# pyannote/pyannote-audio

Measured on AMD Instinct MI355X. Metric: audio-hours/sec (real-time factor) for speaker-diarization-3.1 pipeline, higher is better.
Workload: dtype f32

## Files before the change

### pyannote-audio_amd/csrc/seg_frontend.hip

```cpp
#include "common.h"

namespace pa {

__global__ __launch_bounds__(256) void k_row_stats(const float* __restrict__ x, long row_stride,
                                                    long total_len, int len, float eps,
                                                    float* __restrict__ mean_out,
                                                    float* __restrict__ rstd_out) {
  __shared__ float red[4];
  const long base = (long)blockIdx.x * row_stride;
  long avail = total_len - base;
  int valid = avail >= len ? len : (avail > 0 ? (int)avail : 0);
  const float* row = x + base;
  float s = 0.f;
  for (int i = threadIdx.x; i < valid; i += 256) s += row[i];
  const float mean = block_sum<4>(s, red) / (float)len;
  float q = 0.f;
  for (int i = threadIdx.x; i < valid; i += 256) {
    float d = row[i] - mean;
    q += d * d;
  }
  float var = block_sum<4>(q, red);
  var += (float)(len - valid) * mean * mean;
  var /= (float)len;
  if (threadIdx.x == 0) {
    mean_out[blockIdx.x] = mean;
    rstd_out[blockIdx.x] = 1.0f / sqrtf(var + eps);
  }
}

constexpr int SINC_PT = 128;
constexpr int SINC_XS = 30 * SINC_PT + 256;
constexpr int SINC_OS = SINC_PT + 4;
constexpr int SINC_T = 640;
constexpr float SINC_DEMOTE = 0.5f;

__device__ __forceinline__ float sinc_centre(float mean0, float rstd0) {
  return fabsf(mean0) * rstd0 > SINC_DEMOTE ? mean0 : 0.f;
}
__device__ __forceinline__ bool sinc_demoted(float mu, float rstd, float m0) {
  return fabsf(mu - m0) * rstd > SINC_DEMOTE;
}

template <bool RAW, int STR = 10>
__global__ __launch_bounds__(SINC_T) void k_sinc_fir_pool(
    const float* __restrict__ wav, long wav_len, long chunk_stride, int N, int stride, int P,
    const float* __restrict__ mean, const float* __restrict__ rstd, float gamma, float beta,
    const float* __restrict__ filt, float* __restrict__ out, int centred) {
  constexpr int XS_MAX = 3 * STR * SINC_PT + 256;
  extern __shared__ __attribute__((aligned(16))) float smem[];
  float* xs = smem;
  float* os = smem + XS_MAX;
  const int b = blockIdx.y;
  const int p0 = blockIdx.x * SINC_PT;
  const int tid = threadIdx.x, lane = tid & 63;
  const int w = (tid >> 6) % 5, half = (tid >> 6) / 5;
  constexpr int PS = RAW ? STR : 3 * STR;
  constexpr int XS = RAW ? STR * SINC_PT + 256 : XS_MAX;

  const long cbase = (long)b * chunk_stride;
  if (!RAW && centred && !sinc_demoted(mean[b], rstd[b], sinc_centre(mean[0], rstd[0]))) return;
  const float mu = RAW ? (centred ? sinc_centre(mean[0], rstd[0]) : 0.f) : mean[b], rs = RAW ? 1.f : rstd[b] * gamma;
  if (RAW) beta = 0.f;
  {
    constexpr int NS = (XS_MAX + SINC_T - 1) / SINC_T;
    float raw[NS];
#pragma unroll
    for (int k = 0; k < NS; ++k) {
      const int i = tid + SINC_T * k;
      const long g = cbase + PS * p0 + i;
      raw[k] = (i < XS && PS * p0 + i < N && g < wav_len) ? wav[g] : 0.f;
    }
#pragma unroll
    for (int k = 0; k < NS; ++k) {
      const int i = tid + SINC_T * k;
      if (i < XS) xs[i] = PS * p0 + i < N ? (raw[k] - mu) * rs + beta : 0.f;
    }
  }
  float fb[63];
#pragma unroll
  for (int kt = 0; kt < 63; ++kt) fb[kt] = filt[(w * 63 + kt) * 64 + lane];
  __syncthreads();

  const int i16 = lane & 15, kq = lane >> 4;
#pragma unroll 1
  for (int grp = half * (SINC_PT / 32); grp < (half + 1) * (SINC_PT / 32); ++grp) {
    f32x4 a0 = {0, 0, 0, 0}, a1 = {0, 0, 0, 0}, a2 = {0, 0, 0, 0};
    const float* xp = xs + PS * (16 * grp + i16) + kq;
#pragma unroll
    for (int kt = 0; kt < 63; ++kt) {
      a0 = MFMA16(xp[4 * kt], fb[kt], a0);
      if (!RAW) {
        a1 = MFMA16(xp[4 * kt + STR], fb[kt], a1);
        a2 = MFMA16(xp[4 * kt + 2 * STR], fb[kt], a2);
      }
    }
#pragma unroll
    for (int r = 0; r < 4; ++r) {
      const float v = RAW ? a0[r] : fmaxf(fmaxf(fabsf(a0[r]), fabsf(a1[r])), fabsf(a2[r]));
      os[(16 * w + i16) * SINC_OS + 16 * grp + 4 * kq + r] = v;
    }
  }
  __syncthreads();
  const int np = min(SINC_PT, P - p0);
  for (int i = tid; i < 80 * SINC_PT; i += SINC_T) {
    const int c = i / SINC_PT, p = i % SINC_PT;
    if (p < np) out[((long)b * 80 + c) * P + p0 + p] = os[c * SINC_OS + p];
  }
}

__global__ __launch_bounds__(128) void k_sinc_tapsum(const float* __restrict__ filt, float* __restrict__ S1) {
  const int f = threadIdx.x;
  if (f >= 80) return;
  double acc = 0.0;
  for (int kt = 0; kt < 63; ++kt)
    for (int q = 0; q < 4; ++q) acc += (double)filt[((f >> 4) * 63 + kt) * 64 + (f & 15) + 16 * q];
  S1[f] = (float)acc;
}

__global__ __launch_bounds__(256) void k_sinc_fix_pool(const float* __restrict__ S, long Pc, int Q, int P,
                                                        const float* __restrict__ mean,
                                                        const float* __restrict__ rstd, float gamma, float beta,
                                                        const float* __restrict__ S1, float* __restrict__ out,
                                                        int centred) {
  const int b = blockIdx.y, p = blockIdx.x * 256 + threadIdx.x;
  if (p >= P) return;
  const float m0 = centred ? sinc_centre(mean[0], rstd[0]) : 0.f;
  if (centred && sinc_demoted(mean[b], rstd[b], m0)) return;
  const float mu = mean[b] - m0, g = rstd[b] * gamma;
  const float* src = S + (long)b * Q + 3 * p;
  float* dst = out + (long)b * 80 * P + p;
#pragma unroll 8
  for (int f = 0; f < 80; ++f) {
    const float s1 = S1[f], off = beta * s1 - g * mu * s1;
    const float* row = src + (long)f * Pc;
    const float v0 = fabsf(fmaf(g, row[0], off)), v1 = fabsf(fmaf(g, row[1], off)), v2 = fabsf(fmaf(g, row[2], off));
    dst[(long)f * P] = fmaxf(fmaxf(v0, v1), v2);
  }
}

constexpr int CV_PT = 32;
constexpr int CV_XW = 112;
constexpr int CV_OS = CV_PT + 1;

template <int CIN>
__global__ __launch_bounds__(256) void k_conv5_pool(const float* __restrict__ xin, int Lin, int P,
                                                     const float* __restrict__ in_mean,
                                                     const float* __restrict__ in_rstd,
                                                     const float* __restrict__ gam,
                                                     const float* __restrict__ bet,
                                                     const float* __restrict__ wp,
                                                     const float* __restrict__ bias,
                                                     float* __restrict__ out) {
  constexpr int KT = 5 * CIN / 4;
  constexpr int KPT = CIN / 4;
  __shared__ __attribute__((aligned(16))) float xs[CIN * CV_XW];
  __shared__ float os[64 * CV_OS];
  const int b = blockIdx.y;
  const int p0 = blockIdx.x * CV_PT;
  const int tid = threadIdx.x, lane = tid & 63, w = tid >> 6;

  {
    static_assert(CIN % 20 == 0, "five channel rows per wave and trip");
    const int wu = __builtin_amdgcn_readfirstlane(w);
    const int q1 = lane + 64;
    const bool ok0 = 3 * p0 + lane < Lin;
    const bool ok1 = q1 < 3 * CV_PT + 4 && 3 * p0 + q1 < Lin;
#pragma unroll
    for (int j0 = 0; j0 < CIN / 4; j0 += 5) {
      float x0[5], x1[5], mu[5], sc[5], sh[5];
#pragma unroll
      for (int u = 0; u < 5; ++u) {
        const int c = wu + 4 * (j0 + u), row = b * CIN + c;
        const float* src = xin + (long)row * Lin + 3 * p0;
        x0[u] = ok0 ? src[lane] : 0.f;
        x1[u] = ok1 ? src[q1] : 0.f;
        mu[u] = in_mean[row];
        sc[u] = in_rstd[row] * gam[c];
        sh[u] = bet[c];
      }
#pragma unroll
      for (int u = 0; u < 5; ++u) {
        float* dst = xs + (wu + 4 * (j0 + u)) * CV_XW;
        dst[lane] = ok0 ? leaky_relu((x0[u] - mu[u]) * sc[u] + sh[u]) : 0.f;
        if (q1 < CV_XW) dst[q1] = ok1 ? leaky_relu((x1[u] - mu[u]) * sc[u] + sh[u]) : 0.f;
      }
    }
  }
  float wb[KT];
#pragma unroll
  for (int kt = 0; kt < KT; ++kt) wb[kt] = wp[(w * KT + kt) * 64 + lane];
  __syncthreads();

  const int i16 = lane & 15, kq = lane >> 4;
  const float bv = bias[16 * w + i16];
#pragma unroll 1
  for (int grp = 0; grp < CV_PT / 16; ++grp) {
    f32x4 a0 = {0, 0, 0, 0}, a1 = {0, 0, 0, 0}, a2 = {0, 0, 0, 0};
    const float* xp = xs + kq * CV_XW + 3 * (16 * grp + i16);
#pragma unroll
    for (int kt = 0; kt < KT; ++kt) {
      const int tap = kt / KPT, c4 = (kt % KPT) * 4;
      const float* q = xp + c4 * CV_XW + tap;
      a0 = MFMA16(q[0], wb[kt], a0);
      a1 = MFMA16(q[1], wb[kt], a1);
      a2 = MFMA16(q[2], wb[kt], a2);
    }
#pragma unroll
    for (int r = 0; r < 4; ++r) {
      float v = fmaxf(fmaxf(a0[r], a1[r]), a2[r]) + bv;
      os[(16 * w + i16) * CV_OS + 16 * grp + 4 * kq + r] = v;
    }
  }
  __syncthreads();
  const int np = min(CV_PT, P - p0);
  for (int i = tid; i < 60 * CV_PT; i += 256) {
    const int c = i / CV_PT, p = i % CV_PT;
    if (p < np) out[((long)b * 60 + c) * P + p0 + p] = os[c * CV_OS + p];
  }
}

__global__ __launch_bounds__(256) void k_norm_transpose(const float* __restrict__ xin, int B, int T,
                                                         const float* __restrict__ in_mean,
                                                         const float* __restrict__ in_rstd,
                                                         const float* __restrict__ gam,
                                                         const float* __restrict__ bet,
                                                         float* __restrict__ X0) {
  __shared__ float tile[64][65];
  const int b = blockIdx.y, t0 = blockIdx.x * 64;
  const int tid = threadIdx.x;
  for (int i = tid; i < 64 * 64; i += 256) {
    const int c = i >> 6, tt = i & 63;
    float v = 0.f;
    if (b < B && c < 60 && t0 + tt < T) {
      const int row = b * 60 + c;
      v = (xin[(long)row * T + t0 + tt] - in_mean[row]) * (in_rstd[row] * gam[c]) + bet[c];
      v = leaky_relu(v);
    }
    tile[c][tt] = v;
  }
  __syncthreads();
  const int bt = b >> 4, b16 = b & 15;
  for (int i = tid; i < 64 * 64; i += 256) {
    const int tt = i >> 6, c = i & 63;
    if (t0 + tt < T) X0[(((long)bt * T + t0 + tt) * 16 + b16) * 64 + c] = tile[c][tt];
  }
}

}

extern "C" {

int pa_row_stats(const float* x, long row_stride, long total_len, int rows, int len, float eps,
                 float* mean, float* rstd, void* stream) {
  if (rows <= 0) return 0;
  pa::ProfScope prof("k_row_stats", stream, 5.0 * rows * len, 8.0 * rows * len);
  hipLaunchKernelGGL(pa::k_row_stats, dim3(rows), dim3(256), 0, (hipStream_t)stream, x, row_stride,
                     total_len, len, eps, mean, rstd);
  PA_CHECK_LAUNCH("pa_row_stats");
  return 0;
}

int pa_sinc_fir_pool(const float* wav, long wav_len, long chunk_stride, int B, int N, int stride,
                     const float* mean, const float* rstd, float gamma, float beta,
                     const float* filt_packed, float* out, void* stream) {
  PA_REQUIRE(stride >= 1 && N >= 251, "pa_sinc_fir_pool: stride %d / %d samples", stride, N);
  const int L = (N - 251) / stride + 1;
  const int P = L / 3;
  if (B <= 0 || P <= 0) return 0;
  pa::ProfScope prof("k_sinc_fir_pool", stream, 2.0 * B * 80 * 251 * (3.0 * P),
                     4.0 * B * N + 4.0 * B * 80 * P);
#define PA_SINC_LAUNCH(S)                                                                                          \
  do {                                                                                                             \
    const size_t lds = (size_t)(3 * (S) * pa::SINC_PT + 256 + 80 * pa::SINC_OS) * sizeof(float);                     \
                         \
    (void)hipFuncSetAttribute((const void*)pa::k_sinc_fir_pool<false, S>, hipFuncAttributeMaxDynamicSharedMemorySize, \
                              (int)lds);                                                                           \
    hipLaunchKernelGGL((pa::k_sinc_fir_pool<false, S>), dim3(pa::cdiv(P, pa::SINC_PT), B), dim3(pa::SINC_T), lds,  \
                       (hipStream_t)stream, wav, wav_len, chunk_stride, N, stride, P, mean, rstd, gamma, beta,      \
                       filt_packed, out, 0);                                                                       \
  } while (0)
  switch (stride) {
    case 10: PA_SINC_LAUNCH(10); break;
    case 1: PA_SINC_LAUNCH(1); break;
    case 2: PA_SINC_LAUNCH(2); break;
    case 4: PA_SINC_LAUNCH(4); break;
    case 5: PA_SINC_LAUNCH(5); break;
    case 8: PA_SINC_LAUNCH(8); break;
    case 16: PA_SINC_LAUNCH(16); break;
    case 20: PA_SINC_LAUNCH(20); break;
    default:
      PA_REQUIRE(false, "pa_sinc_fir_pool: SincNet stride %d is not built (1, 2, 4, 5, 8, 10, 16, 20 are)", stride);
  }
#undef PA_SINC_LAUNCH
  PA_CHECK_LAUNCH("pa_sinc_fir_pool");
  return 0;
}

static int sinc_fir_span(const float* wav, long wav_len, long span, const float* mean0, const float* rstd0,
                         const float* filt_packed, float* S, void* stream) {
  if (span < 251) return 0;
  PA_REQUIRE(span <= 0x7fffffffL, "pa_sinc_fir_span: span of %ld samples is too long", span);
  const int Pc = (int)((span - 251) / 10 + 1);
  const size_t lds = (pa::SINC_XS + 80 * pa::SINC_OS) * sizeof(float);
  (void)hipFuncSetAttribute((const void*)pa::k_sinc_fir_pool<true>, hipFuncAttributeMaxDynamicSharedMemorySize,
                            (int)lds);
  pa::ProfScope prof("k_sinc_fir_span", stream, 2.0 * 80 * 251 * (double)Pc, 4.0 * span + 4.0 * 80 * Pc);
  hipLaunchKernelGGL(pa::k_sinc_fir_pool<true>, dim3(pa::cdiv(Pc, pa::SINC_PT), 1), dim3(pa::SINC_T), lds,
                     (hipStream_t)stream, wav, wav_len, 0L, (int)span, 10, Pc, mean0, rstd0, 1.f, 0.f, filt_packed, S,
                     mean0 != nullptr ? 1 : 0);
  PA_CHECK_LAUNCH("pa_sinc_fir_span");
  return 0;
}

int pa_sinc_fir_span(const float* wav, long wav_len, long span, const float* filt_packed, float* S, void* stream) {
  return sinc_fir_span(wav, wav_len, span, nullptr, nullptr, filt_packed, S, stream);
}

int pa_sinc_fir_span_centred(const float* wav, long wav_len, long span, const float* mean0, const float* rstd0,
                             const float* filt_packed, float* S, void* stream) {
  PA_REQUIRE(mean0 != nullptr && rstd0 != nullptr, "pa_sinc_fir_span_centred: the statistics of chunk 0 are missing");
  return sinc_fir_span(wav, wav_len, span, mean0, rstd0, filt_packed, S, stream);
}

int pa_sinc_fix_pool(const float* S, long Pc, int positions_per_chunk_step, int B, int P, const float* mean,
                     const float* rstd, float gamma, float beta, const float* filt_packed, float* tap_sums,
                     float* out, void* stream) {
  if (B <= 0 || P <= 0) return 0;
  pa::ProfScope prof("k_sinc_fix_pool", stream, 8.0 * B * 80 * 3.0 * P, 4.0 * B * 80 * 4.0 * P);
  hipLaunchKernelGGL(pa::k_sinc_tapsum, dim3(1), dim3(128), 0, (hipStream_t)stream, filt_packed, tap_sums);
  hipLaunchKernelGGL(pa::k_sinc_fix_pool, dim3(pa::cdiv(P, 256), B), dim3(256), 0, (hipStream_t)stream, S, Pc,
                     positions_per_chunk_step, P, mean, rstd, gamma, beta, (const float*)tap_sums, out, 0);
  PA_CHECK_LAUNCH("pa_sinc_fix_pool");
  return 0;
}

int pa_sinc_fix_pool_centred(const float* S, long Pc, int positions_per_chunk_step, int B, int P, const float* wav,
                             long wav_len, int N, const float* mean, const float* rstd, float gamma, float beta,
                             const float* filt_packed, float* tap_sums, float* out, void* stream) {
  if (B <= 0 || P <= 0) return 0;
  PA_REQUIRE(N >= 251 && P == ((N - 251) / 10 + 1) / 3, "pa_sinc_fix_pool_centred: %d pooled positions of %d samples",
             P, N);
  pa::ProfScope prof("k_sinc_fix_pool", stream, 8.0 * B * 80 * 3.0 * P, 4.0 * B * 80 * 4.0 * P);
  hipLaunchKernelGGL(pa::k_sinc_tapsum, dim3(1), dim3(128), 0, (hipStream_t)stream, filt_packed, tap_sums);
  hipLaunchKernelGGL(pa::k_sinc_fix_pool, dim3(pa::cdiv(P, 256), B), dim3(256), 0, (hipStream_t)stream, S, Pc,
                     positions_per_chunk_step, P, mean, rstd, gamma, beta, (const float*)tap_sums, out, 1);
  {
    const size_t lds = (pa::SINC_XS + 80 * pa::SINC_OS) * sizeof(float);
    (void)hipFuncSetAttribute((const void*)pa::k_sinc_fir_pool<false, 10>, hipFuncAttributeMaxDynamicSharedMemorySize,
                              (int)lds);
    hipLaunchKernelGGL((pa::k_sinc_fir_pool<false, 10>), dim3(pa::cdiv(P, pa::SINC_PT), B), dim3(pa::SINC_T), lds,
                       (hipStream_t)stream, wav, wav_len, 10L * positions_per_chunk_step, N, 10, P, mean, rstd, gamma,
                       beta, filt_packed, out, 1);
  }
  PA_CHECK_LAUNCH("pa_sinc_fix_pool_centred");
  return 0;
}

int pa_conv5_pool(const float* xin, int B, int cin, int Lin, const float* in_mean,
                  const float* in_rstd, const float* gam, const float* bet, const float* w_packed,
                  const float* bias64, float* out, void* stream) {
  const int P = (Lin - 4) / 3;
  if (B <= 0 || P <= 0) return 0;
  dim3 grid(pa::cdiv(P, pa::CV_PT), B);
  pa::ProfScope prof("k_conv5_pool", stream, 2.0 * B * 60 * cin * 5 * (3.0 * P),
                     4.0 * B * cin * Lin + 4.0 * B * 60 * P);
  if (cin == 80)
    hipLaunchKernelGGL(pa::k_conv5_pool<80>, grid, dim3(256), 0, (hipStream_t)stream, xin, Lin, P,
                       in_mean, in_rstd, gam, bet, w_packed, bias64, out);
  else if (cin == 60)
    hipLaunchKernelGGL(pa::k_conv5_pool<60>, grid, dim3(256), 0, (hipStream_t)stream, xin, Lin, P,
                       in_mean, in_rstd, gam, bet, w_packed, bias64, out);
  else
    PA_REQUIRE(false, "pa_conv5_pool: unsupported cin %d", cin);
  PA_CHECK_LAUNCH("pa_conv5_pool");
  return 0;
}

int pa_norm_transpose(const float* xin, int B, int T, const float* in_mean, const float* in_rstd,
                      const float* gam, const float* bet, float* X0, void* stream) {
  if (B <= 0) return 0;
  const int ntiles = (B + 15) / 16;
  pa::ProfScope prof("k_norm_transpose", stream, 4.0 * B * 60 * T, 4.0 * B * 60 * T + 4.0 * ntiles * 16 * 64 * T);
  hipLaunchKernelGGL(pa::k_norm_transpose, dim3(pa::cdiv(T, 64), ntiles * 16), dim3(256), 0,
                     (hipStream_t)stream, xin, B, T, in_mean, in_rstd, gam, bet, X0);
  PA_CHECK_LAUNCH("pa_norm_transpose");
  return 0;
}

}
```

### pyannote-audio_amd/csrc/seg_lstm.hip

```cpp
#include "common.h"

namespace pa {

constexpr int GB = 128;
constexpr int GK = 32;
constexpr int GLD = GK + 4;

template <int ACT, int OUT_MODE>
__global__ __launch_bounds__(256) void k_gemm_tn(const float* __restrict__ A, int lda,
                                                  const float* __restrict__ W, int ldw,
                                                  const float* __restrict__ bias,
                                                  const float* __restrict__ Res,
                                                  float* __restrict__ C, long ldc, int M, int N, int K,
                                                  int nm, int nn, int inner, long sAo, long sAi, long sWo,
                                                  long sWi, long sCo, long sCi, int gHW, int gWo, int gH, int gW) {
  if (gridDim.y > 1) {
    const int zo = blockIdx.y / inner, zi = blockIdx.y % inner;
    A += zo * sAo + zi * sAi;
    W += zo * sWo + zi * sWi;
    C += zo * sCo + zi * sCi;
    if (Res != nullptr) Res += zo * sCo + zi * sCi;
  }
  __shared__ __attribute__((aligned(16))) float As[GB * GLD];
  __shared__ __attribute__((aligned(16))) float Ws[GB * GLD];
  int mt, nt;
  const int bid = blockIdx.x;
  if (nn == 8) {
    nt = (bid >> 3) & 7;
    mt = (bid & 7) + 8 * (bid >> 6);
  } else {
    nt = bid % nn;
    mt = bid / nn;
  }
  if (mt >= nm) return;
  const int m0 = mt * GB, n0 = nt * GB;
  const int tid = threadIdx.x, lane = tid & 63, wv = tid >> 6;
  const int wm = wv >> 1, wn = wv & 1;
  const int lr = tid >> 3, lc = (tid & 7) * 4;

  float4 ra[4], rw[4];
  const float* ap[4];
  const float* wp[4];
#pragma unroll
  for (int i = 0; i < 4; ++i) {
    const int ar = m0 + lr + 32 * i, wr = n0 + lr + 32 * i;
    long arow = ar;
    if (gHW > 0) {
      const int b = ar / gHW, rem = ar - b * gHW, y = rem / gWo, x = rem - y * gWo;
      arow = ((long)b * gH + 2 * y) * gW + 2 * x;
    }
    ap[i] = ar < M ? A + arow * lda + lc : nullptr;
    wp[i] = wr < N ? W + (long)wr * ldw + lc : nullptr;
  }
  auto gload = [&](int k0) {
#pragma unroll
    for (int i = 0; i < 4; ++i) {
      ra[i] = ap[i] != nullptr ? *reinterpret_cast<const float4*>(ap[i] + k0) : make_float4(0.f, 0.f, 0.f, 0.f);
      rw[i] = wp[i] != nullptr ? *reinterpret_cast<const float4*>(wp[i] + k0) : make_float4(0.f, 0.f, 0.f, 0.f);
    }
  };
  auto lstore = [&]() {
#pragma unroll
    for (int i = 0; i < 4; ++i) {
      *reinterpret_cast<float4*>(As + (lr + 32 * i) * GLD + lc) = ra[i];
      *reinterpret_cast<float4*>(Ws + (lr + 32 * i) * GLD + lc) = rw[i];
    }
  };

  f32x16 acc[2][2];
#pragma unroll
  for (int i = 0; i < 2; ++i)
#pragma unroll
    for (int j = 0; j < 2; ++j)
#pragma unroll
      for (int r = 0; r < 16; ++r) acc[i][j][r] = 0.f;

  const int fi = lane & 31, kh = lane >> 5;
  gload(0);
  for (int k0 = 0; k0 < K; k0 += GK) {
    __syncthreads();
    lstore();
    __syncthreads();
    if (k0 + GK < K) gload(k0 + GK);
#pragma unroll
    for (int r4 = 0; r4 < 4; ++r4) {
      float4 af[2], wf[2];
#pragma unroll
      for (int i = 0; i < 2; ++i) {
        af[i] = *reinterpret_cast<const float4*>(As + (64 * wm + 32 * i + fi) * GLD + kh * 16 + 4 * r4);
        wf[i] = *reinterpret_cast<const float4*>(Ws + (64 * wn + 32 * i + fi) * GLD + kh * 16 + 4 * r4);
      }
#pragma unroll
      for (int i = 0; i < 2; ++i)
#pragma unroll
        for (int j = 0; j < 2; ++j) {
          acc[i][j] = MFMA32(af[i].x, wf[j].x, acc[i][j]);
          acc[i][j] = MFMA32(af[i].y, wf[j].y, acc[i][j]);
          acc[i][j] = MFMA32(af[i].z, wf[j].z, acc[i][j]);
          acc[i][j] = MFMA32(af[i].w, wf[j].w, acc[i][j]);
        }
    }
  }

#pragma unroll
  for (int i = 0; i < 2; ++i)
#pragma unroll
    for (int j = 0; j < 2; ++j) {
      const int n = n0 + 64 * wn + 32 * j + fi;
      const float bv = (bias != nullptr && n < N) ? bias[n] : 0.f;
#pragma unroll
      for (int q = 0; q < 4; ++q) {
        const int m = m0 + 64 * wm + 32 * i + 8 * q + 4 * kh;
        float v[4];
#pragma unroll
        for (int e = 0; e < 4; ++e) {
          v[e] = acc[i][j][4 * q + e] + bv;
          if (OUT_MODE == 0 && Res != nullptr && n < N && m + e < M) v[e] += Res[(long)(m + e) * ldc + n];
          if (ACT == 1) v[e] = leaky_relu(v[e]);
          if (ACT == 2) v[e] = fmaxf(v[e], 0.f);
          if (ACT == 3) v[e] = gelu_erf(v[e]);
        }
        if (n < N) {
          if (OUT_MODE == 0) {
#pragma unroll
            for (int e = 0; e < 4; ++e)
              if (m + e < M) C[(long)(m + e) * ldc + n] = v[e];
          } else {
            if (m < M)
              *reinterpret_cast<float4*>(C + ((long)(m >> 4) * N + n) * 16 + (m & 15)) =
                  make_float4(v[0], v[1], v[2], v[3]);
          }
        }
      }
    }
}

constexpr int LSTM_HS = 162;

__device__ __forceinline__ float sigmoidf_(float x) {
  return __builtin_amdgcn_rcpf(1.0f + __builtin_amdgcn_exp2f(-1.4426950408889634f * x));
}
__device__ __forceinline__ float tanhf_(float x) {
  const float xc = fminf(fmaxf(x, -15.f), 15.f);
  return 2.0f * __builtin_amdgcn_rcpf(1.0f + __builtin_amdgcn_exp2f(-2.8853900817779268f * xc)) - 1.0f;
}

__global__ __launch_bounds__(256, 1) void k_lstm_rec(const float* __restrict__ xproj,
                                                      const float* __restrict__ whh_p,
                                                      float* __restrict__ out, int T) {
  __shared__ float hs[2 * 16 * LSTM_HS];
  const int tile = blockIdx.x, dir = blockIdx.y;
  const int tid = threadIdx.x, lane = tid & 63, w = tid >> 6;
  const int n = lane & 15, g = lane >> 4;

  float wr[8][32];
  {
    const float* wp = whh_p + (long)((dir * 4 + w) * 8 * 32) * 64 + lane;
#pragma unroll
    for (int q8 = 0; q8 < 8; ++q8)
#pragma unroll
      for (int kt = 0; kt < 32; ++kt) wr[q8][kt] = wp[(q8 * 32 + kt) * 64];
  }
  for (int i = tid; i < 2 * 16 * LSTM_HS; i += 256) hs[i] = 0.f;
  float c[2][4];
#pragma unroll
  for (int s = 0; s < 2; ++s)
#pragma unroll
    for (int r = 0; r < 4; ++r) c[s][r] = 0.f;
  __syncthreads();

  const float* xbase = xproj + ((long)tile * T * 1024 + dir * 512 + w * 128 + n) * 16 + 4 * g;
  float* obase = out + ((long)tile * T * 16 + 4 * g) * 256 + dir * 128 + 32 * w + n;

  f32x4 xin[8];
  {
    const int t = dir ? T - 1 : 0;
#pragma unroll
    for (int q8 = 0; q8 < 8; ++q8)
      xin[q8] = *reinterpret_cast<const f32x4*>(xbase + ((long)t * 1024 + q8 * 16) * 16);
  }
  int cur = 0;
#pragma unroll 1
  for (int step = 0; step < T; ++step) {
    const int t = dir ? T - 1 - step : step;
    f32x4 acc[8];
#pragma unroll
    for (int q8 = 0; q8 < 8; ++q8) acc[q8] = xin[q8];
    if (step + 1 < T) {
      const int tn = dir ? t - 1 : t + 1;
#pragma unroll
      for (int q8 = 0; q8 < 8; ++q8)
        xin[q8] = *reinterpret_cast<const f32x4*>(xbase + ((long)tn * 1024 + q8 * 16) * 16);
    }
    const float* hp = hs + (cur * 16 + n) * LSTM_HS + g * 33;
    float a[32];
#pragma unroll
    for (int kt = 0; kt < 32; ++kt) a[kt] = hp[kt];
#pragma unroll
    for (int kt = 0; kt < 32; ++kt)
#pragma unroll
      for (int q8 = 0; q8 < 8; ++q8) acc[q8] = MFMA16(a[kt], wr[q8][kt], acc[q8]);

    float* hn = hs + ((cur ^ 1) * 16 + 4 * g) * LSTM_HS + w * 33 + n;
    float* op = obase + (long)t * 16 * 256;
#pragma unroll
    for (int s = 0; s < 2; ++s)
#pragma unroll
      for (int r = 0; r < 4; ++r) {
        const float ig = sigmoidf_(acc[0 + s][r]);
        const float fg = sigmoidf_(acc[2 + s][r]);
        const float gg = tanhf_(acc[4 + s][r]);
        const float og = sigmoidf_(acc[6 + s][r]);
        const float cn = fg * c[s][r] + ig * gg;
        c[s][r] = cn;
        const float h = og * tanhf_(cn);
        hn[r * LSTM_HS + 16 * s] = h;
        op[r * 256 + 16 * s] = h;
      }
    __syncthreads();
    cur ^= 1;
  }
}

constexpr int LSTMG_MT = 2;
constexpr int LSTMG_MAXU = 8;

__global__ __launch_bounds__(256) void k_lstm_rec_gen(const float* __restrict__ xproj,
                                                      const float* __restrict__ whh_g,
                                                      float* __restrict__ out, int T, int H, int ntiles,
                                                      int ndir, int hstride) {
  extern __shared__ float hsg[];
  constexpr int MT = LSTMG_MT;
  const int tile0 = blockIdx.x * MT, dir = blockIdx.y;
  const int tid = threadIdx.x, lane = tid & 63, w = tid >> 6;
  const int n = lane & 15, g = lane >> 4;
  const int U = H >> 4, K4 = H >> 4;
  const long NG = (long)ndir * 4 * H;
  const int ldo = ndir * H;
  for (int i = tid; i < MT * 2 * 16 * hstride; i += 256) hsg[i] = 0.f;
  f32x4 c[LSTMG_MAXU][MT];
#pragma unroll
  for (int ui = 0; ui < LSTMG_MAXU; ++ui)
#pragma unroll
    for (int mt = 0; mt < MT; ++mt) c[ui][mt] = f32x4{0.f, 0.f, 0.f, 0.f};
  __syncthreads();
  int tl[MT];
  bool live[MT];
#pragma unroll
  for (int mt = 0; mt < MT; ++mt) {
    live[mt] = tile0 + mt < ntiles;
    tl[mt] = live[mt] ? tile0 + mt : ntiles - 1;
  }
  int cur = 0;
#pragma unroll 1
  for (int step = 0; step < T; ++step) {
    const int t = dir ? T - 1 - step : step;
#pragma unroll
    for (int ui = 0; ui < LSTMG_MAXU; ++ui) {
      const int u = w + 4 * ui;
      if (u >= U) break;
      f32x4 xin[MT][4], acc[MT][4];
#pragma unroll
      for (int mt = 0; mt < MT; ++mt)
#pragma unroll
        for (int q = 0; q < 4; ++q) {
          xin[mt][q] = *reinterpret_cast<const f32x4*>(
              xproj + (((long)tl[mt] * T + t) * NG + (long)dir * 4 * H + (4 * u + q) * 16 + n) * 16 + 4 * g);
          acc[mt][q] = f32x4{0.f, 0.f, 0.f, 0.f};
        }
      const f32x4* wp = reinterpret_cast<const f32x4*>(whh_g) + ((long)(dir * U + u) * 4 * K4) * 64 + lane;
      const float* hp0 = hsg + (cur * 16 + n) * hstride + g;
#pragma unroll 2
      for (int k4 = 0; k4 < K4; ++k4) {
        f32x4 b[4];
#pragma unroll
        for (int q = 0; q < 4; ++q) b[q] = wp[(long)(q * K4 + k4) * 64];
#pragma unroll
        for (int j = 0; j < 4; ++j) {
#pragma unroll
          for (int mt = 0; mt < MT; ++mt) {
            const float a = hp0[mt * 2 * 16 * hstride + 16 * k4 + 4 * j];
#pragma unroll
            for (int q = 0; q < 4; ++q) acc[mt][q] = MFMA16(a, b[q][j], acc[mt][q]);
          }
        }
      }
#pragma unroll
      for (int mt = 0; mt < MT; ++mt) {
        float* hn = hsg + ((mt * 2 + (cur ^ 1)) * 16 + 4 * g) * hstride + 16 * u + n;
        float* op = out + (((long)tl[mt] * T + t) * 16 + 4 * g) * ldo + dir * H + 16 * u + n;
#pragma unroll
        for (int r = 0; r < 4; ++r) {
          const float ig = sigmoidf_(acc[mt][0][r] + xin[mt][0][r]);
          const float fg = sigmoidf_(acc[mt][1][r] + xin[mt][1][r]);
          const float gg = tanhf_(acc[mt][2][r] + xin[mt][2][r]);
          const float og = sigmoidf_(acc[mt][3][r] + xin[mt][3][r]);
          const float cn = fg * c[ui][mt][r] + ig * gg;
          c[ui][mt][r] = cn;
          const float h = og * tanhf_(cn);
          hn[r * hstride] = h;
          if (live[mt]) op[(long)r * ldo] = h;
        }
      }
    }
    __syncthreads();
    cur ^= 1;
  }
}

constexpr int CLS_MAXC = 16;

__global__ __launch_bounds__(256) void k_classifier(const float* __restrict__ X, int ldx, int K, int M,
                                                     int T, int B, const float* __restrict__ cw,
                                                     const float* __restrict__ cb, int NC,
                                                     const unsigned char* __restrict__ mapping, int S,
                                                     float* __restrict__ logp,
                                                     unsigned char* __restrict__ ml) {
  extern __shared__ float wsh[];
  for (int i = threadIdx.x; i < NC * K; i += 256) wsh[i] = cw[i];
  for (int i = threadIdx.x; i < NC; i += 256) wsh[NC * K + i] = cb[i];
  __syncthreads();
  const long m = (long)blockIdx.x * 256 + threadIdx.x;
  if (m >= M) return;
  const int b16 = (int)(m & 15);
  const long tt = m >> 4;
  const int t = (int)(tt % T), tile = (int)(tt / T);
  const int b = tile * 16 + b16;
  if (b >= B) return;
  float z[CLS_MAXC];
#pragma unroll
  for (int cidx = 0; cidx < CLS_MAXC; ++cidx) z[cidx] = cidx < NC ? wsh[NC * K + cidx] : 0.f;
  const float* x = X + m * ldx;
  for (int k = 0; k < K; k += 4) {
    const float4 xv = *reinterpret_cast<const float4*>(x + k);
#pragma unroll
    for (int cidx = 0; cidx < CLS_MAXC; ++cidx)
      if (cidx < NC) {
        const float* wrow = wsh + cidx * K + k;
        z[cidx] = fmaf(xv.x, wrow[0], z[cidx]);
        z[cidx] = fmaf(xv.y, wrow[1], z[cidx]);
        z[cidx] = fmaf(xv.z, wrow[2], z[cidx]);
        z[cidx] = fmaf(xv.w, wrow[3], z[cidx]);
      }
  }
  const long o = (long)b * T + t;
  if (mapping == nullptr) {
    if (logp != nullptr)
      for (int cidx = 0; cidx < NC; ++cidx) logp[o * NC + cidx] = 1.f / (1.f + expf(-z[cidx]));
    return;
  }
  float mx = z[0];
  int am = 0;
#pragma unroll
  for (int cidx = 1; cidx < CLS_MAXC; ++cidx)
    if (cidx < NC && z[cidx] > mx) {
      mx = z[cidx];
      am = cidx;
    }
  float se = 0.f;
#pragma unroll
  for (int cidx = 0; cidx < CLS_MAXC; ++cidx)
    if (cidx < NC) se += expf(z[cidx] - mx);
  const float lse = mx + logf(se);
  if (logp != nullptr)
    for (int cidx = 0; cidx < NC; ++cidx) logp[o * NC + cidx] = z[cidx] - lse;
  if (ml != nullptr)
    for (int s = 0; s < S; ++s) ml[o * S + s] = mapping[am * S + s];
}

}

extern "C" {

int pa_gemm_tn_ex(const float* A, int lda, const float* W, int ldw, const float* bias, const float* Res,
                  float* C, long ldc, int M, int N, int K, int act, int out_mode, void* stream);

int pa_gemm_tn(const float* A, int lda, const float* W, int ldw, const float* bias, float* C, long ldc,
               int M, int N, int K, int act, int out_mode, void* stream) {
  return pa_gemm_tn_ex(A, lda, W, ldw, bias, nullptr, C, ldc, M, N, K, act, out_mode, stream);
}

int pa_gemm_tn_batched(const float* A, int lda, long sAo, long sAi, const float* W, int ldw, long sWo, long sWi,
                       const float* bias, float* C, long ldc, long sCo, long sCi, int M, int N, int K,
                       int outer, int inner, int act, void* stream);

static int gemm_tn_launch(const float* A, int lda, const float* W, int ldw, const float* bias, const float* Res,
                          float* C, long ldc, int M, int N, int K, int act, int out_mode, int gHW, int gWo, int gH,
                          int gW, void* stream);

int pa_gemm_tn_ex(const float* A, int lda, const float* W, int ldw, const float* bias, const float* Res,
                  float* C, long ldc, int M, int N, int K, int act, int out_mode, void* stream) {
  return gemm_tn_launch(A, lda, W, ldw, bias, Res, C, ldc, M, N, K, act, out_mode, 0, 0, 0, 0, stream);
}

int pa_gemm_tn_s2(const float* X, int B, int H, int W, int cin, const float* Wt, int ldw, const float* bias, float* C,
                  long ldc, int N, void* stream) {
  const int Ho = (H - 1) / 2 + 1, Wo = (W - 1) / 2 + 1;
  if (B <= 0) return 0;
  return gemm_tn_launch(X, cin, Wt, ldw, bias, nullptr, C, ldc, B * Ho * Wo, N, cin, 0, 0, Ho * Wo, Wo, H, W, stream);
}

static int gemm_tn_launch(const float* A, int lda, const float* W, int ldw, const float* bias, const float* Res,
                          float* C, long ldc, int M, int N, int K, int act, int out_mode, int gHW, int gWo, int gH,
                          int gW, void* stream) {
  if (M <= 0 || N <= 0) return 0;
  PA_REQUIRE(Res == nullptr || out_mode == 0, "pa_gemm_tn_ex: a residual needs out_mode 0");
  PA_REQUIRE(K % pa::GK == 0 && lda % 4 == 0 && ldw % 4 == 0,
             "pa_gemm_tn: K (%d) must be a multiple of 32 and lda/ldw multiples of 4", K);
  PA_REQUIRE(out_mode == 0 || (M % 16 == 0), "pa_gemm_tn: out_mode 1 needs M %% 16 == 0");
  const int nm = pa::cdiv(M, pa::GB), nn = pa::cdiv(N, pa::GB);
  const int grid = nn == 8 ? pa::cdiv(nm, 8) * 64 : nm * nn;
  hipStream_t st = (hipStream_t)stream;
  pa::ProfScope prof("k_gemm_tn", stream, 2.0 * M * N * K, 4.0 * ((double)M * K + (double)N * K + (double)M * N));
#define PA_GEMM(ACT, OM)                                                                          \
  hipLaunchKernelGGL((pa::k_gemm_tn<ACT, OM>), dim3(grid), dim3(256), 0, st, A, lda, W, ldw, bias, \
                     Res, C, ldc, M, N, K, nm, nn, 1, 0L, 0L, 0L, 0L, 0L, 0L, gHW, gWo, gH, gW)
  if (act == 0 && out_mode == 0) PA_GEMM(0, 0);
  else if (act == 1 && out_mode == 0) PA_GEMM(1, 0);
  else if (act == 2 && out_mode == 0) PA_GEMM(2, 0);
  else if (act == 3 && out_mode == 0) PA_GEMM(3, 0);
  else if (act == 0 && out_mode == 1) PA_GEMM(0, 1);
  else PA_REQUIRE(false, "pa_gemm_tn: unsupported act/out_mode %d/%d", act, out_mode);
#undef PA_GEMM
  PA_CHECK_LAUNCH("pa_gemm_tn");
  return 0;
}

int pa_gemm_tn_batched(const float* A, int lda, long sAo, long sAi, const float* W, int ldw, long sWo, long sWi,
                       const float* bias, float* C, long ldc, long sCo, long sCi, int M, int N, int K,
                       int outer, int inner, int act, void* stream) {
  if (M <= 0 || N <= 0 || outer <= 0 || inner <= 0) return 0;
  PA_REQUIRE(K % pa::GK == 0 && lda % 4 == 0 && ldw % 4 == 0 && sAo % 4 == 0 && sAi % 4 == 0 && sWo % 4 == 0 &&
                 sWi % 4 == 0,
             "pa_gemm_tn_batched: K (%d) must be a multiple of 32 and every stride a multiple of 4", K);
  PA_REQUIRE((long)outer * inner <= 65535, "pa_gemm_tn_batched: at most 65535 products per launch");
  const int nm = pa::cdiv(M, pa::GB), nn = pa::cdiv(N, pa::GB);
  const int grid = nn == 8 ? pa::cdiv(nm, 8) * 64 : nm * nn;
  hipStream_t st = (hipStream_t)stream;
  const double z = (double)outer * inner;
  pa::ProfScope prof("k_gemm_tn", stream, 2.0 * z * M * N * K, 4.0 * z * ((double)M * K + (double)N * K + (double)M * N));
#define PA_GEMMB(ACT)                                                                                          \
  hipLaunchKernelGGL((pa::k_gemm_tn<ACT, 0>), dim3(grid, outer * inner), dim3(256), 0, st, A, lda, W, ldw, bias, \
                     (const float*)nullptr, C, ldc, M, N, K, nm, nn, inner, sAo, sAi, sWo, sWi, sCo, sCi, 0, 0, 0, 0)
  if (act == 0) PA_GEMMB(0);
  else if (act == 3) PA_GEMMB(3);
  else PA_REQUIRE(false, "pa_gemm_tn_batched: unsupported act %d", act);
#undef PA_GEMMB
  PA_CHECK_LAUNCH("pa_gemm_tn_batched");
  return 0;
}

int pa_lstm_rec(const float* xproj, const float* whh_packed, float* out, int ntiles, int ndir, int T,
                void* stream) {
  if (ntiles <= 0 || T <= 0) return 0;
  pa::ProfScope prof("k_lstm_rec", stream, 2.0 * ntiles * 16 * ndir * T * 128 * 512,
                     4.0 * ntiles * 16 * ndir * T * (512 + 128));
  hipLaunchKernelGGL(pa::k_lstm_rec, dim3(ntiles, ndir), dim3(256), 0, (hipStream_t)stream, xproj,
                     whh_packed, out, T);
  PA_CHECK_LAUNCH("pa_lstm_rec");
  return 0;
}

int pa_lstm_rec_h(const float* xproj, const float* whh_packed, float* out, int ntiles, int ndir, int T, int H,
                  void* stream) {
  if (ntiles <= 0 || T <= 0) return 0;
  if (H == 128 && ndir == 2) return pa_lstm_rec(xproj, whh_packed, out, ntiles, ndir, T, stream);
  PA_REQUIRE(H >= 16 && H % 16 == 0 && H <= 64 * pa::LSTMG_MAXU && (ndir == 1 || ndir == 2),
             "pa_lstm_rec_h: hidden size %d must be a multiple of 16 in [16, %d], directions 1 or 2 (got %d)", H,
             64 * pa::LSTMG_MAXU, ndir);
  const int hstride = ((H + 63) / 64) * 64 + 4;
  const size_t lds = sizeof(float) * pa::LSTMG_MT * 2 * 16 * hstride;
  {
    int dev = 0, limit = 0;
    (void)hipGetDevice(&dev);
    (void)hipDeviceGetAttribute(&limit, hipDeviceAttributeMaxSharedMemoryPerBlock, dev);
    PA_REQUIRE(limit <= 0 || lds <= (size_t)limit,
               "pa_lstm_rec_h: hidden size %d needs %zu bytes of LDS per workgroup, this device offers %d", H, lds, limit);
    static size_t granted = 0;
    if (lds > granted) {
      PA_REQUIRE(hipFuncSetAttribute((const void*)pa::k_lstm_rec_gen, hipFuncAttributeMaxDynamicSharedMemorySize,
                                     (int)lds) == hipSuccess,
                 "pa_lstm_rec_h: cannot reserve %zu bytes of dynamic LDS for hidden size %d", lds, H);
      granted = lds;
    }
  }
  pa::ProfScope prof("k_lstm_rec_gen", stream, 2.0 * ntiles * 16 * ndir * T * H * 4.0 * H,
                     4.0 * ntiles * 16 * ndir * T * (4.0 * H + H));
  hipLaunchKernelGGL(pa::k_lstm_rec_gen, dim3(pa::cdiv(ntiles, pa::LSTMG_MT), ndir), dim3(256), lds,
                     (hipStream_t)stream, xproj, whh_packed, out, T, H, ntiles, ndir, hstride);
  PA_CHECK_LAUNCH("pa_lstm_rec_h");
  return 0;
}

int pa_classifier(const float* X, int ldx, int K, int ntiles, int T, int B, const float* cw,
                  const float* cb, int NC, const unsigned char* mapping, int S, float* logp,
                  unsigned char* multilabel, void* stream) {
  PA_REQUIRE(NC <= pa::CLS_MAXC && K % 4 == 0, "pa_classifier: NC <= 16 and K %% 4 == 0 required");
  const long M = (long)ntiles * T * 16;
  if (M <= 0) return 0;
  const size_t lds = (size_t)(NC * K + NC) * sizeof(float);
  pa::ProfScope prof("k_classifier", stream, 2.0 * M * K * NC, 4.0 * M * K + 4.0 * M * NC);
  hipLaunchKernelGGL(pa::k_classifier, dim3(pa::cdiv(M, 256)), dim3(256), lds, (hipStream_t)stream, X,
                     ldx, K, (int)M, T, B, cw, cb, NC, mapping, S, logp, multilabel);
  PA_CHECK_LAUNCH("pa_classifier");
  return 0;
}

}
```

Baseline: 1.346.

## Register-cache row stats and software-pipeline LDS loads in LSTM recurrence

Row statistics now keep each row's elements in registers across the mean and variance passes. This removes the second global read, using a templated unroll count picked from the row length. The LSTM recurrent kernel now streams the hidden state from LDS in double-buffered chunks of four, interleaved with the MFMAs under sched_barriers, and issues the next-step input prefetch after the first chunk. It also replaces __syncthreads with a barrier that waits only on LDS counters, so the global output stores are not drained each step. The lighter barrier relies on correct memory-ordering assumptions, and the register caching raises register pressure.

```diff
diff --git a/pyannote-audio_amd/csrc/seg_frontend.hip b/pyannote-audio_amd/csrc/seg_frontend.hip
--- a/pyannote-audio_amd/csrc/seg_frontend.hip
+++ b/pyannote-audio_amd/csrc/seg_frontend.hip
@@ -1,7 +1,10 @@
+#include <stdlib.h>
+
 #include "common.h"
 
 namespace pa {
 
+template <int NV>
 __global__ __launch_bounds__(256) void k_row_stats(const float* __restrict__ x, long row_stride,
                                                     long total_len, int len, float eps,
                                                     float* __restrict__ mean_out,
@@ -11,13 +14,37 @@
   long avail = total_len - base;
   int valid = avail >= len ? len : (avail > 0 ? (int)avail : 0);
   const float* row = x + base;
+  constexpr int NR = NV > 0 ? NV : 1;
+  float v[NR];
+  if (NV > 0) {
+#pragma unroll
+    for (int k = 0; k < NR; ++k) {
+      const int i = threadIdx.x + 256 * k;
+      v[k] = i < valid ? row[i] : 0.f;
+    }
+  }
   float s = 0.f;
-  for (int i = threadIdx.x; i < valid; i += 256) s += row[i];
+  if (NV > 0) {
+#pragma unroll
+    for (int k = 0; k < NR; ++k)
+      if ((int)threadIdx.x + 256 * k < valid) s += v[k];
+  } else {
+    for (int i = threadIdx.x; i < valid; i += 256) s += row[i];
+  }
   const float mean = block_sum<4>(s, red) / (float)len;
   float q = 0.f;
-  for (int i = threadIdx.x; i < valid; i += 256) {
-    float d = row[i] - mean;
-    q += d * d;
+  if (NV > 0) {
+#pragma unroll
+    for (int k = 0; k < NR; ++k)
+      if ((int)threadIdx.x + 256 * k < valid) {
+        float d = v[k] - mean;
+        q += d * d;
+      }
+  } else {
+    for (int i = threadIdx.x; i < valid; i += 256) {
+      float d = row[i] - mean;
+      q += d * d;
+    }
   }
   float var = block_sum<4>(q, red);
   var += (float)(len - valid) * mean * mean;
@@ -254,8 +281,19 @@
                  float* mean, float* rstd, void* stream) {
   if (rows <= 0) return 0;
   pa::ProfScope prof("k_row_stats", stream, 5.0 * rows * len, 8.0 * rows * len);
-  hipLaunchKernelGGL(pa::k_row_stats, dim3(rows), dim3(256), 0, (hipStream_t)stream, x, row_stride,
-                     total_len, len, eps, mean, rstd);
+  const char* e = getenv("PA_ROW_STATS_REGS");
+  const int nv = (e == nullptr || atoi(e) != 0) ? pa::cdiv(len, 256) : 25;
+#define PA_RS(NV)                                                                                                   \
+  hipLaunchKernelGGL(pa::k_row_stats<NV>, dim3(rows), dim3(256), 0, (hipStream_t)stream, x, row_stride, total_len, len, \
+                     eps, mean, rstd)
+  if (nv <= 1) PA_RS(1);
+  else if (nv <= 3) PA_RS(3);
+  else if (nv <= 7) PA_RS(7);
+  else if (nv <= 12) PA_RS(12);
+  else if (nv <= 21) PA_RS(21);
+  else if (nv <= 24) PA_RS(24);
+  else PA_RS(0);
+#undef PA_RS
   PA_CHECK_LAUNCH("pa_row_stats");
   return 0;
 }
diff --git a/pyannote-audio_amd/csrc/seg_lstm.hip b/pyannote-audio_amd/csrc/seg_lstm.hip
--- a/pyannote-audio_amd/csrc/seg_lstm.hip
+++ b/pyannote-audio_amd/csrc/seg_lstm.hip
@@ -145,6 +145,12 @@
   return 2.0f * __builtin_amdgcn_rcpf(1.0f + __builtin_amdgcn_exp2f(-2.8853900817779268f * xc)) - 1.0f;
 }
 
+__device__ __forceinline__ void lstm_step_barrier() {
+  asm volatile("s_waitcnt lgkmcnt(0)" ::: "memory");
+  __builtin_amdgcn_s_barrier();
+  asm volatile("" ::: "memory");
+}
+
 __global__ __launch_bounds__(256, 1) void k_lstm_rec(const float* __restrict__ xproj,
                                                       const float* __restrict__ whh_p,
                                                       float* __restrict__ out, int T) {
@@ -178,28 +184,38 @@
 #pragma unroll
     for (int q8 = 0; q8 < 8; ++q8)
       xin[q8] = *reinterpret_cast<const f32x4*>(xbase + ((long)t * 1024 + q8 * 16) * 16);
+#pragma unroll
+    for (int q8 = 0; q8 < 8; ++q8) asm volatile("" : "+v"(xin[q8]));
   }
   int cur = 0;
 #pragma unroll 1
   for (int step = 0; step < T; ++step) {
     const int t = dir ? T - 1 - step : step;
+    const int tn = step + 1 < T ? (dir ? t - 1 : t + 1) : t;
     f32x4 acc[8];
-#pragma unroll
-    for (int q8 = 0; q8 < 8; ++q8) acc[q8] = xin[q8];
-    if (step + 1 < T) {
-      const int tn = dir ? t - 1 : t + 1;
-#pragma unroll
-      for (int q8 = 0; q8 < 8; ++q8)
-        xin[q8] = *reinterpret_cast<const f32x4*>(xbase + ((long)tn * 1024 + q8 * 16) * 16);
-    }
     const float* hp = hs + (cur * 16 + n) * LSTM_HS + g * 33;
-    float a[32];
-#pragma unroll
-    for (int kt = 0; kt < 32; ++kt) a[kt] = hp[kt];
-#pragma unroll
-    for (int kt = 0; kt < 32; ++kt)
-#pragma unroll
-      for (int q8 = 0; q8 < 8; ++q8) acc[q8] = MFMA16(a[kt], wr[q8][kt], acc[q8]);
+    float a[2][4];
+#pragma unroll
+    for (int k = 0; k < 4; ++k) a[0][k] = hp[k];
+#pragma unroll
+    for (int ch = 0; ch < 8; ++ch) {
+      if (ch + 1 < 8) {
+#pragma unroll
+        for (int k = 0; k < 4; ++k) a[(ch + 1) & 1][k] = hp[4 * (ch + 1) + k];
+      }
+      __builtin_amdgcn_sched_barrier(0);
+#pragma unroll
+      for (int k = 0; k < 4; ++k)
+#pragma unroll
+        for (int q8 = 0; q8 < 8; ++q8)
+          acc[q8] = MFMA16(a[ch & 1][k], wr[q8][4 * ch + k], (ch == 0 && k == 0) ? xin[q8] : acc[q8]);
+      __builtin_amdgcn_sched_barrier(0);
+      if (ch == 0) {
+#pragma unroll
+        for (int q8 = 0; q8 < 8; ++q8)
+          xin[q8] = *reinterpret_cast<const f32x4*>(xbase + ((long)tn * 1024 + q8 * 16) * 16);
+      }
+    }
 
     float* hn = hs + ((cur ^ 1) * 16 + 4 * g) * LSTM_HS + w * 33 + n;
     float* op = obase + (long)t * 16 * 256;
@@ -211,13 +227,13 @@
         const float fg = sigmoidf_(acc[2 + s][r]);
         const float gg = tanhf_(acc[4 + s][r]);
         const float og = sigmoidf_(acc[6 + s][r]);
-        const float cn = fg * c[s][r] + ig * gg;
+        const float cn = fmaf(ig, gg, fg * c[s][r]);
         c[s][r] = cn;
         const float h = og * tanhf_(cn);
         hn[r * LSTM_HS + 16 * s] = h;
         op[r * 256 + 16 * s] = h;
       }
-    __syncthreads();
+    lstm_step_barrier();
     cur ^= 1;
   }
 }
```

New measurement: 1.354 (median of 6 runs). About the same (+0.6%).
